# hugofloresgarcia/vampnet

Measured on NVIDIA H100. Metric: codec tokens/sec (coarse 12 steps + c2f 24 steps generate, T=768, 44.1 kHz), higher is better.
Workload: dtype bf16

## Files before the change

vampnet_b200/csrc/api.cu:

```cuda
#include <cuda_bf16.h>
#include <cudaTypedefs.h>

#include <cmath>
#include <cstdarg>
#include <cstdio>
#include <cstring>
#include <map>
#include <memory>
#include <string>
#include <tuple>
#include <vector>

#include "kernels.h"

namespace vnb {

static thread_local std::string g_err;
static thread_local std::string g_tmap_err;

static int fail(const char* fmt, ...) {
  char buf[1024];
  va_list ap;
  va_start(ap, fmt);
  vsnprintf(buf, sizeof(buf), fmt, ap);
  va_end(ap);
  g_err = buf;
  return 1;
}
#define CK(expr)                                                                                   \
  do {                                                                                             \
    cudaError_t _e = (expr);                                                                       \
    if (_e != cudaSuccess) return fail("%s failed: %s (%s:%d)", #expr, cudaGetErrorString(_e), __FILE__, __LINE__); \
  } while (0)

static PFN_cuTensorMapEncodeTiled_v12000 get_encode() {
  static PFN_cuTensorMapEncodeTiled_v12000 fn = nullptr;
  if (fn) return fn;
  void* p = nullptr;
  cudaDriverEntryPointQueryResult q;
  cudaError_t e = cudaGetDriverEntryPoint("cuTensorMapEncodeTiled", &p, cudaEnableDefault, &q);
  if (e != cudaSuccess || q != cudaDriverEntryPointSuccess || !p) {
    g_tmap_err = std::string("cudaGetDriverEntryPoint(cuTensorMapEncodeTiled) failed: ") + cudaGetErrorString(e);
    return nullptr;
  }
  fn = reinterpret_cast<PFN_cuTensorMapEncodeTiled_v12000>(p);
  return fn;
}
const char* tmap_error() { return g_tmap_err.c_str(); }

bool make_tmap_2d(CUtensorMap* tm, const void* base, uint64_t rows, uint64_t cols, uint32_t box_rows,
                  uint32_t box_cols) {
  auto enc = get_encode();
  if (!enc) return false;
  cuuint64_t dims[2] = {cols, rows};
  cuuint64_t strides[1] = {cols * 2};
  cuuint32_t box[2] = {box_cols, box_rows};
  cuuint32_t estr[2] = {1, 1};
  CUresult r = enc(tm, CU_TENSOR_MAP_DATA_TYPE_BFLOAT16, 2, const_cast<void*>(base), dims, strides, box, estr,
                   CU_TENSOR_MAP_INTERLEAVE_NONE, CU_TENSOR_MAP_SWIZZLE_128B, CU_TENSOR_MAP_L2_PROMOTION_L2_256B,
                   CU_TENSOR_MAP_FLOAT_OOB_FILL_NONE);
  if (r != CUDA_SUCCESS) {
    char b[256];
    snprintf(b, sizeof(b), "cuTensorMapEncodeTiled(2d rows=%llu cols=%llu box=%ux%u) -> %d", (unsigned long long)rows,
             (unsigned long long)cols, box_rows, box_cols, (int)r);
    g_tmap_err = b;
    return false;
  }
  return true;
}
bool make_tmap_3d(CUtensorMap* tm, const void* base, uint64_t batch, uint64_t rows, uint64_t cols,
                  uint64_t pitch_elems, uint32_t box_rows, uint32_t box_cols) {
  auto enc = get_encode();
  if (!enc) return false;
  cuuint64_t dims[3] = {cols, rows, batch};
  cuuint64_t strides[2] = {pitch_elems * 2, rows * pitch_elems * 2};
  cuuint32_t box[3] = {box_cols, box_rows, 1};
  cuuint32_t estr[3] = {1, 1, 1};
  CUresult r = enc(tm, CU_TENSOR_MAP_DATA_TYPE_BFLOAT16, 3, const_cast<void*>(base), dims, strides, box, estr,
                   CU_TENSOR_MAP_INTERLEAVE_NONE, CU_TENSOR_MAP_SWIZZLE_128B, CU_TENSOR_MAP_L2_PROMOTION_L2_256B,
                   CU_TENSOR_MAP_FLOAT_OOB_FILL_NONE);
  if (r != CUDA_SUCCESS) {
    char b[256];
    snprintf(b, sizeof(b), "cuTensorMapEncodeTiled(3d batch=%llu rows=%llu cols=%llu pitch=%llu box=%ux%u) -> %d",
             (unsigned long long)batch, (unsigned long long)rows, (unsigned long long)cols,
             (unsigned long long)pitch_elems, box_rows, box_cols, (int)r);
    g_tmap_err = b;
    return false;
  }
  return true;
}

static bool make_gemm_plan(GemmPlan* p, int epi, const void* A, const void* W, int M, int N, int K, void* out,
                           void* out2, const float* bias, int T, int Tpad, const float* ss_in, int ss_parts,
                           float inv_d, float eps, void* out_bf16, float* ss_out) {
  if (N % 256 != 0 || K % 64 != 0 || M < 1) {
    g_tmap_err = "gemm: need N % 256 == 0 and K % 64 == 0";
    return false;
  }
  GemmArgs& a = p->args;
  a.M = M; a.N = N; a.K = K; a.epi = epi; a.out = out; a.out2 = out2; a.bias = bias;
  a.T = T; a.Tpad = Tpad; a.d2 = epi == VNB_EPI_QKV ? (N / 3) * 2 : 0;
  if (ss_in != nullptr) { a.ss_in = ss_in; a.ss_parts = ss_parts; a.inv_d = inv_d; a.eps = eps; }
  a.out_bf16 = reinterpret_cast<__nv_bfloat16*>(out_bf16); a.ss_out = ss_out;
  return make_tmap_2d(&p->tmA, A, M, K, 128, 64) && make_tmap_2d(&p->tmB, W, N, K, 256, 64) &&
         make_tmap_2d(&p->tmBh, W, N, K, 128, 64);
}

bool make_attn_plan(AttnPlan* p, const void* qk, const void* vT, void* out, const float* rel, int sat, int B, int T,
                    int Tpad, int H) {
  const int d = H * 64;
  p->out = out; p->rel = rel; p->sat = sat; p->B = B; p->T = T; p->Tpad = Tpad; p->H = H;
  return make_tmap_3d(&p->tmQ, qk, B, T, 2 * d, 2 * d, 128, 64) && make_tmap_3d(&p->tmK, qk, B, T, 2 * d, 2 * d, 64, 64) &&
         make_tmap_3d(&p->tmVT, vT, B, d, Tpad, Tpad, 64, 64);
}

struct DevBuf {
  void* p = nullptr;
  size_t n = 0;
  ~DevBuf() { if (p) cudaFree(p); }
  cudaError_t alloc(size_t bytes, bool zero = false) {
    n = bytes;
    cudaError_t e = cudaMalloc(&p, bytes ? bytes : 1);
    if (e == cudaSuccess && zero) e = cudaMemset(p, 0, bytes);
    return e;
  }
  template <class T> T* as() const { return reinterpret_cast<T*>(p); }
};

struct Variant {
  int steps = 0;
  bool has_mask = false;
  bool top_p = false;
  int gemm_pair = 0;
  bool fused = false;
  bool adapted = false;
  bool ragged = false;
  bool mixed_steps = false;
  bool split = false;
  bool operator<(const Variant& o) const {
    return std::tie(steps, has_mask, top_p, gemm_pair, fused, adapted, ragged, mixed_steps, split) <
           std::tie(o.steps, o.has_mask, o.top_p, o.gemm_pair, o.fused, o.adapted, o.ragged, o.mixed_steps, o.split);
  }
};

struct Workspace {
  int B = 0, T = 0, Tpad = 0, M = 0;
  unsigned long long last_use = 0;
  DevBuf x, y, qk, vT, att, h, logits, zcur, zorig, tokens, conf, n0, dyn, rowgrp, z_in, mask_in, z_out, ssA, ssB, embA,
      partials;
  DevBuf grp_adapter, lora_u;
  DevBuf frames;
  DevBuf live;
  int embKp = 0;
  int ss_parts = 0;
  std::vector<GemmPlan> qkv, wo, up, down;
  GemmPlan cls, emb;
  GemmPlan cls_sample;
  bool can_fuse = false;
  AttnPlan attn;
  std::map<Variant, cudaGraphExec_t> graphs;
  std::map<Variant, unsigned long long> graph_kernels;
  ~Workspace() { for (auto& kv : graphs) cudaGraphExecDestroy(kv.second); }
};

}

namespace vnb {
enum { FAM_EMBED = 0, FAM_RMSNORM, FAM_GEMM_QKV, FAM_ATTN, FAM_GEMM_O, FAM_GEMM_UP, FAM_GEMM_DOWN, FAM_GEMM_CLS,
       FAM_SAMPLE, FAM_STATE, FAM_LORA_DOWN, FAM_COUNT };
static unsigned long long g_captures = 0;
static unsigned long long g_launches = 0;
void count_launch(unsigned long long n) { g_launches += n; }
struct Profiler {
  bool on = false;
  std::vector<cudaEvent_t> pool;
  std::vector<int> fam;
  size_t used = 0;
  ~Profiler() { for (auto e : pool) cudaEventDestroy(e); }
  void mark(int family, cudaStream_t st) {
    if (!on) return;
    if (used == pool.size()) {
      cudaEvent_t e;
      if (cudaEventCreate(&e) != cudaSuccess) { on = false; return; }
      pool.push_back(e);
      fam.push_back(-1);
    }
// ... 1133 lines not shown
```

vampnet_b200/csrc/common.cuh:

```cuda
#pragma once
#include <cuda.h>
#include <cuda_bf16.h>
#include <cuda_runtime.h>
#include <stdint.h>
#include <stdio.h>

namespace vnb {

__device__ __forceinline__ uint32_t smem_u32(const void* p) {
  return static_cast<uint32_t>(__cvta_generic_to_shared(p));
}
__device__ __forceinline__ uint32_t lane_id() { return threadIdx.x & 31; }

__device__ __forceinline__ bool elect_one() {
  uint32_t pred = 0;
  asm volatile(
      "{\n\t.reg .pred P;\n\t.reg .b32 R;\n\t"
      "elect.sync R|P, 0xffffffff;\n\t"
      "selp.u32 %0, 1, 0, P;\n\t}"
      : "=r"(pred));
  return pred != 0;
}

__device__ __forceinline__ void mbar_init(uint64_t* bar, uint32_t count) {
// ... 91 lines not shown

__device__ __forceinline__ void tma_store_2d(const CUtensorMap* m, const void* src, int c0, int c1) {
  asm volatile("cp.async.bulk.tensor.2d.global.shared::cta.bulk_group [%0, {%2, %3}], [%1];"
               ::"l"(reinterpret_cast<uint64_t>(m)), "r"(smem_u32(src)), "r"(c0), "r"(c1)
               : "memory");
}
__device__ __forceinline__ void bulk_commit() { asm volatile("cp.async.bulk.commit_group;" ::: "memory"); }
template <int N>
__device__ __forceinline__ void bulk_wait_read() {
  asm volatile("cp.async.bulk.wait_group.read %0;" ::"n"(N) : "memory");
}

__device__ __forceinline__ uint32_t cluster_ctarank() {
  uint32_t r;
  asm volatile("mov.u32 %0, %%cluster_ctarank;" : "=r"(r));
  return r;
}
__device__ __forceinline__ void cluster_sync_all() {
  asm volatile("barrier.cluster.arrive.release.aligned;\n\tbarrier.cluster.wait.acquire.aligned;" ::: "memory");
}
__device__ __forceinline__ uint32_t mapa_u32(uint32_t cta_addr, uint32_t rank) {
  uint32_t r;
  asm volatile("mapa.shared::cluster.u32 %0, %1, %2;" : "=r"(r) : "r"(cta_addr), "r"(rank));
  return r;
}
__device__ __forceinline__ void mbar_arrive_cluster(uint32_t cluster_addr) {
  asm volatile("mbarrier.arrive.release.cluster.shared::cluster.b64 _, [%0];" ::"r"(cluster_addr) : "memory");
}
__device__ __forceinline__ bool mbar_try_wait_cluster(uint64_t* bar, uint32_t parity) {
  uint32_t ok;
  asm volatile(
      "{\n\t.reg .pred P;\n\t"
      "mbarrier.try_wait.parity.acquire.cluster.shared::cta.b64 P, [%1], %2, %3;\n\t"
      "selp.u32 %0, 1, 0, P;\n\t}"
      : "=r"(ok)
      : "r"(smem_u32(bar)), "r"(parity), "r"(100000u)
      : "memory");
  return ok != 0;
}
__device__ __forceinline__ void mbar_wait_cluster(uint64_t* bar, uint32_t parity) {
  if (mbar_try_wait_cluster(bar, parity)) return;
  const uint64_t t0 = global_timer_ns();
  while (!mbar_try_wait_cluster(bar, parity))
    if (global_timer_ns() - t0 > VNB_WAIT_TIMEOUT_NS) __trap();
}
__device__ __forceinline__ void tma_load_2d_mc(void* dst, const CUtensorMap* m, uint64_t* bar, int c0, int c1,
                                               uint16_t cta_mask) {
  asm volatile(
      "cp.async.bulk.tensor.2d.shared::cluster.global.mbarrier::complete_tx::bytes.multicast::cluster"
      " [%0], [%1, {%3, %4}], [%2], %5;"
      ::"r"(smem_u32(dst)), "l"(reinterpret_cast<uint64_t>(m)), "r"(smem_u32(bar)), "r"(c0), "r"(c1), "h"(cta_mask)
      : "memory");
}

__device__ __forceinline__ uint32_t pack_bf16x2(float lo, float hi) {
  __nv_bfloat162 v = __floats2bfloat162_rn(lo, hi);
  return *reinterpret_cast<uint32_t*>(&v);
}
__device__ __forceinline__ float fast_exp2(float x) {
  float y;
  asm volatile("ex2.approx.ftz.f32 %0, %1;" : "=f"(y) : "f"(x));
  return y;
}
__device__ __forceinline__ float lds_f32(uint32_t addr) {
  float v;
  asm volatile("ld.shared.f32 %0, [%1];" : "=f"(v) : "r"(addr));
  return v;
}
__device__ __forceinline__ void sts_f32(uint32_t addr, float v) {
  asm volatile("st.shared.f32 [%0], %1;" ::"r"(addr), "f"(v) : "memory");
}
__device__ __forceinline__ void sts_u32(uint32_t addr, uint32_t v) {
  asm volatile("st.shared.b32 [%0], %1;" ::"r"(addr), "r"(v) : "memory");
}
__device__ __forceinline__ float4 lds_f4(uint32_t addr) {
  float4 v;
  asm volatile("ld.shared.v4.f32 {%0, %1, %2, %3}, [%4];" : "=f"(v.x), "=f"(v.y), "=f"(v.z), "=f"(v.w) : "r"(addr));
  return v;
}
__device__ __forceinline__ uint2 lds_u2(uint32_t addr) {
  uint2 v;
  asm volatile("ld.shared.v2.b32 {%0, %1}, [%2];" : "=r"(v.x), "=r"(v.y) : "r"(addr));
  return v;
}
__device__ __forceinline__ void sts_f4(uint32_t addr, float4 v) {
  asm volatile("st.shared.v4.f32 [%0], {%1, %2, %3, %4};" ::"r"(addr), "f"(v.x), "f"(v.y), "f"(v.z), "f"(v.w)
               : "memory");
}
__device__ __forceinline__ void sts_v4(uint32_t addr, uint32_t a, uint32_t b, uint32_t c, uint32_t d) {
  asm volatile("st.shared.v4.b32 [%0], {%1, %2, %3, %4};" ::"r"(addr), "r"(a), "r"(b), "r"(c), "r"(d) : "memory");
}
__device__ __forceinline__ float warp_max(float v) {
#pragma unroll
  for (int o = 16; o > 0; o >>= 1) v = fmaxf(v, __shfl_xor_sync(0xffffffffu, v, o));
  return v;
}
__device__ __forceinline__ float warp_sum(float v) {
#pragma unroll
  for (int o = 16; o > 0; o >>= 1) v += __shfl_xor_sync(0xffffffffu, v, o);
  return v;
}

__device__ __forceinline__ void philox4x32_10(uint32_t c0, uint32_t c1, uint32_t c2, uint32_t c3, uint32_t k0,
                                              uint32_t k1, uint32_t (&out)[4]) {
#pragma unroll
  for (int r = 0; r < 10; ++r) {
    const uint32_t hi0 = __umulhi(0xD2511F53u, c0), lo0 = 0xD2511F53u * c0;
    const uint32_t hi1 = __umulhi(0xCD9E8D57u, c2), lo1 = 0xCD9E8D57u * c2;
    const uint32_t n0 = hi1 ^ c1 ^ k0, n2 = hi0 ^ c3 ^ k1;
    c0 = n0; c1 = lo1; c2 = n2; c3 = lo0;
    k0 += 0x9E3779B9u;
    k1 += 0xBB67AE85u;
  }
  out[0] = c0; out[1] = c1; out[2] = c2; out[3] = c3;
}
__device__ __forceinline__ float u01(uint32_t x) { return (static_cast<float>(x >> 9) + 0.5f) * 1.1920928955078125e-07f; }

}
```

vampnet_b200/csrc/gemm_wgmma.cu:

```cuda
#include <stdlib.h>

#include "common.cuh"
#include "kernels.h"
#include "wgmma.cuh"

#ifndef VNB_GEMM_PAIR_DEFAULT
#define VNB_GEMM_PAIR_DEFAULT false
#endif

namespace vnb {

constexpr int BM = 128, BN = 256, BK = 64, STAGES = 4;
constexpr int A_BYTES = BM * BK * 2;
constexpr int B_BYTES = BN * BK * 2;
constexpr int STAGE_BYTES = A_BYTES + B_BYTES;
constexpr int SBIAS_BYTES = BN * 4;
constexpr int RING_BYTES = STAGES * STAGE_BYTES;
constexpr int ACC_PITCH = BN + 1;
static_assert(BM * ACC_PITCH * 4 <= RING_BYTES, "the accumulator tile overlays the ring");
static_assert(BM * ACC_PITCH * 4 + 4 * BM + 16 + 32 * BM <= RING_BYTES, "the adapted epilogue's row table follows it");
constexpr int GEMM_SMEM = RING_BYTES + SBIAS_BYTES + 1024  + 256 ;
static_assert(GEMM_SMEM <= 227 * 1024, "H100: at most 227 KiB of shared memory per block");
constexpr int GEMM_THREADS = 256 + 32;
template <int EPI> constexpr int gemm_epi_warps() { return (EPI == VNB_EPI_RESID || EPI == VNB_EPI_SAMPLE) ? 8 : 4; }
// ... 381 lines not shown
              for (int j4 = 0; j4 < 8; ++j4) {
                const float4 b4 = lds_f4(sb4 + 16u * (c * 8 + j4));
                const float bj[4] = {b4.x, b4.y, b4.z, b4.w};
#pragma unroll
                for (int j = 0; j < 4; ++j) {
                  const float x = __fadd_rn(__fmul_rn(__uint_as_float(v[j4 * 4 + j]), rs), bj[j]);
                  run += fast_exp2(__fmaf_rn(x, c1, c0));
                  if (run > target && found < 0) { found = c * 32 + j4 * 4 + j; xc = x; }
                }
              }
            }
            if (found >= 0) cand = found;
            else xc = mx;
          }
          if (active)
            g.partials[(static_cast<size_t>(row) * Cp + cp) * (g.V >> 7) + (v0 >> 7)] =
                make_float4(mx, ssum, xc, __uint_as_float(static_cast<uint32_t>(v0 + cand) |
                                                          (static_cast<uint32_t>(v0 + am) << 16)));
        }
      } else if constexpr (EPI == VNB_EPI_RESID || EPI == VNB_EPI_BIAS_F32) {
        const bool fused_out = g.out_bf16 != nullptr;
        constexpr int CSTEP = kWide ? 2 : 1;
        float ssacc[8];
#pragma unroll
        for (int i = 0; i < 8; ++i) ssacc[i] = 0.f;
        auto process = [&](int c, const float4 (&add)[8]) {
          if (fused_out) drain_f32<true>(g, qaddr, rs, lane, row_base, n0, c, add, ssacc);
          else drain_f32<false>(g, qaddr, rs, lane, row_base, n0, c, add, ssacc);
        };
        float4 addA[8], addB[8];
        prefetch_addend<EPI>(g, lane, row_base, n0 + half * 32, addA);
#pragma unroll 1
        for (int c = half; c < BN / 32; c += 2 * CSTEP) {
          prefetch_addend<EPI>(g, lane, row_base, n0 + (c + CSTEP) * 32, addB);
          process(c, addA);
          if (c + 2 * CSTEP < BN / 32) prefetch_addend<EPI>(g, lane, row_base, n0 + (c + 2 * CSTEP) * 32, addA);
          process(c + CSTEP, addB);
        }
        if (fused_out) {
#pragma unroll
          for (int it = 0; it < 8; ++it) {
            float v = ssacc[it];
            v += __shfl_xor_sync(0xffffffffu, v, 1);
            v += __shfl_xor_sync(0xffffffffu, v, 2);
            v += __shfl_xor_sync(0xffffffffu, v, 4);
            const int rr = row_base + it * 4 + (lane >> 3);
            const int part = (n0 / BN) * (kWide ? 2 : 1) + half;
            if ((lane & 7) == 0 && rr < g.M) g.ss_out[static_cast<size_t>(part) * g.M + rr] = v;
          }
        }
      } else {
#pragma unroll 1
        for (int c = 0; c < BN / 32; ++c) {
          const int col0 = n0 + c * 32;
          if constexpr (EPI == VNB_EPI_QKV) {
            if (col0 >= g.d2) {
              uint32_t v[32];
              acc_ld_x32(t_addr + 4u * (c * 32), v);
              if (row_ok) {
                const int d = g.N - g.d2;
                __nv_bfloat16* o = reinterpret_cast<__nv_bfloat16*>(g.out2) +
                                   (static_cast<size_t>(b_idx) * d + (col0 - g.d2)) * g.Tpad + t_idx;
                const bool pad = g.frames != nullptr && t_idx >= __ldg(g.frames + b_idx);
#pragma unroll
                for (int j = 0; j < 32; ++j)
                  o[static_cast<size_t>(j) * g.Tpad] =
                      pad ? __float2bfloat16_rn(0.f) : __float2bfloat16_rn(__uint_as_float(v[j]) * rs);
              }
              continue;
            }
          }
          drain_bf16<false>(reinterpret_cast<__nv_bfloat16*>(g.out), EPI == VNB_EPI_BF16 ? g.N : g.d2, g.M, qaddr, rs, lane,
                            row_base, c * 32, col0);
        }
      }
    }
  }
  if constexpr (PAIR) cluster_sync_all();
}

constexpr int PERS_EPI_WARPS = 3;
constexpr int PERS_THREADS = 256 + 32 * PERS_EPI_WARPS + 32;
template <int EPI> constexpr int pers_stages() { return EPI == VNB_EPI_QKV ? 3 : STAGES; }
template <int EPI> constexpr int pers_out_bytes() { return EPI == VNB_EPI_QKV ? BM * BN * 2 : BM * (BN / 2) * 2; }
template <int EPI>
constexpr int pers_smem() {
  return pers_stages<EPI>() * STAGE_BYTES + pers_out_bytes<EPI>() + 4 * BM  + 1024  +
         128 ;
}
static_assert(pers_smem<VNB_EPI_GEGLU>() <= 227 * 1024, "H100: at most 227 KiB of shared memory per block");
static_assert(pers_smem<VNB_EPI_QKV>() <= 227 * 1024, "H100: at most 227 KiB of shared memory per block");
static_assert((2 * STAGES + 2) * 8 <= 128, "the barriers fit their slot");

template <int PITCH>
__device__ __forceinline__ uint32_t stage_off(int r, int w) {
  return static_cast<uint32_t>(r * PITCH + (((w >> 2) ^ (r & 7)) << 4) + ((w & 3) << 2));
}

template <int EPI>
__global__ void __launch_bounds__(PERS_THREADS, 1)
gemm_persistent_kernel(const __grid_constant__ CUtensorMap tmA, const __grid_constant__ CUtensorMap tmB,
                       const GemmArgs g) {
  constexpr int NS = pers_stages<EPI>();
  constexpr int RING = NS * STAGE_BYTES;
  constexpr int OUT_BYTES = pers_out_bytes<EPI>();
  extern __shared__ uint8_t smem_raw[];
  uint8_t* smem = reinterpret_cast<uint8_t*>((reinterpret_cast<uintptr_t>(smem_raw) + 1023) & ~uintptr_t(1023));
  const uint32_t stage_tile = smem_u32(smem + RING);
  float* srs = reinterpret_cast<float*>(smem + RING + OUT_BYTES);
  uint64_t* full_bar = reinterpret_cast<uint64_t*>(smem + RING + OUT_BYTES + 4 * BM);
  uint64_t* empty_bar = full_bar + NS;
  uint64_t* out_full = empty_bar + NS;
  uint64_t* out_free = out_full + 1;

  const int warp = threadIdx.x >> 5;
  const int lane = threadIdx.x & 31;
  const int num_n = g.N / BN;
  const int num_kb = g.K / BK;
  const int tiles = ((live_rows(g) + BM - 1) / BM) * num_n;
  constexpr int kProducer = 8 + PERS_EPI_WARPS;

  if (warp == kProducer && lane == 0) {
    tma_prefetch_desc(&tmA);
    tma_prefetch_desc(&tmB);
    for (int s = 0; s < NS; ++s) {
      mbar_init(&full_bar[s], 1);
      mbar_init(&empty_bar[s], 8);
    }
    mbar_init(out_full, 256);
    mbar_init(out_free, 32 * PERS_EPI_WARPS);
    mbar_fence_init();
  }
  __syncthreads();

  if (warp == kProducer) {
    if (lane == 0) {
      int stage = 0;
      uint32_t phase = 0;
      for (int tile = blockIdx.x; tile < tiles; tile += gridDim.x) {
        const int m0 = (tile / num_n) * BM, n0 = (tile % num_n) * BN;
        for (int kb = 0; kb < num_kb; ++kb) {
          mbar_wait(&empty_bar[stage], phase ^ 1);
          uint8_t* sa = smem + stage * STAGE_BYTES;
          mbar_expect_tx(&full_bar[stage], STAGE_BYTES);
          tma_load_2d(sa, &tmA, &full_bar[stage], kb * BK, m0);
          tma_load_2d(sa + A_BYTES, &tmB, &full_bar[stage], kb * BK, n0);
          if (++stage == NS) { stage = 0; phase ^= 1; }
        }
      }
    }
    __syncwarp();
  } else if (warp < 8) {
    int stage = 0;
    uint32_t phase = 0;
    uint32_t it = 0;
    const int r = (warp >> 2) * 64 + (warp & 3) * 16 + (lane >> 2);
    for (int tile = blockIdx.x; tile < tiles; tile += gridDim.x, ++it) {
      float acc[128];
      gemm_mainloop<NS>(acc, smem, full_bar, num_kb, warp >> 2, stage, phase, [&](int s) {
        if (lane == 0) mbar_arrive(&empty_bar[s]);
      });
      mbar_wait(out_free, it & 1u);
      const float rs0 = srs[r], rs1 = srs[r + 8];
      if constexpr (EPI == VNB_EPI_GEGLU) {
#pragma unroll
        for (int i = 0; i < 16; ++i) {
          float x[4];
#pragma unroll
          for (int k = 0; k < 4; ++k) {
            const float rsr = k < 2 ? rs0 : rs1;
            x[k] = acc[4 * i + k] * rsr;
            x[k] = x[k] * gelu_tanh(acc[4 * (i + 16) + k] * rsr);
          }
          const int w = 4 * i + (lane & 3);
          sts_u32(stage_tile + stage_off<256>(r, w), pack_bf16x2(x[0], x[1]));
          sts_u32(stage_tile + stage_off<256>(r + 8, w), pack_bf16x2(x[2], x[3]));
        }
      } else if ((tile % num_n) * BN < g.d2) {
#pragma unroll
        for (int i = 0; i < 32; ++i) {
          const int w = 4 * i + (lane & 3);
          sts_u32(stage_tile + stage_off<512>(r, w), pack_bf16x2(acc[4 * i] * rs0, acc[4 * i + 1] * rs0));
          sts_u32(stage_tile + stage_off<512>(r + 8, w), pack_bf16x2(acc[4 * i + 2] * rs1, acc[4 * i + 3] * rs1));
        }
      } else {
        const bool odd = (lane >> 2) & 1;
#pragma unroll
        for (int i = 0; i < 32; ++i) {
          const int c = 8 * i + 2 * (lane & 3) + (odd ? 1 : 0);
#pragma unroll
          for (int h = 0; h < 2; ++h) {
            const float rsr = h ? rs1 : rs0;
            const uint32_t own = pack_bf16x2(acc[4 * i + 2 * h] * rsr, acc[4 * i + 2 * h + 1] * rsr);
            const uint32_t peer = __shfl_xor_sync(0xffffffffu, own, 4);
            sts_u32(stage_tile + stage_off<256>(c, (r + 8 * h) >> 1),
                    odd ? __byte_perm(peer, own, 0x7632) : __byte_perm(own, peer, 0x5410));
          }
        }
      }
      mbar_arrive(out_full);
    }
  } else {
    const int e = warp - 8;
    __nv_bfloat16* const out = reinterpret_cast<__nv_bfloat16*>(g.out);
    const int pitch = EPI == VNB_EPI_GEGLU ? g.N / 2 : g.d2;
    auto row_scales = [&](int tile) {
      if (tile < tiles) {
        const int m0 = (tile / num_n) * BM;
        for (int j = e * 32 + lane; j < BM; j += 32 * PERS_EPI_WARPS) srs[j] = row_scale(g, m0 + j);
      }
      mbar_arrive(out_free);
    };
    row_scales(blockIdx.x);
    uint32_t it = 0;
    for (int tile = blockIdx.x; tile < tiles; tile += gridDim.x, ++it) {
      const int m0 = (tile / num_n) * BM, n0 = (tile % num_n) * BN;
      mbar_wait(out_full, it & 1u);
      if constexpr (EPI == VNB_EPI_GEGLU) {
#pragma unroll 4
        for (int u = e; u < BM / 2; u += PERS_EPI_WARPS) {
          const int rr = 2 * u + (lane >> 4);
          const float4 v = lds_f4(stage_tile + stage_off<256>(rr, 4 * (lane & 15)));
          if (m0 + rr < g.M)
            *reinterpret_cast<float4*>(out + static_cast<size_t>(m0 + rr) * pitch + (n0 >> 1) + 8 * (lane & 15)) = v;
        }
      } else if (n0 < g.d2) {
#pragma unroll 4
        for (int rr = e; rr < BM; rr += PERS_EPI_WARPS) {
          const float4 v = lds_f4(stage_tile + stage_off<512>(rr, 4 * lane));
          if (m0 + rr < g.M)
            *reinterpret_cast<float4*>(out + static_cast<size_t>(m0 + rr) * pitch + n0 + 8 * lane) = v;
        }
      } else {
        const int d = g.N - g.d2;
        uint16_t* const vt = reinterpret_cast<uint16_t*>(g.out2) + static_cast<size_t>(n0 - g.d2) * g.Tpad;
        size_t off[4];
        bool ok[4];
        int bk[4];
        uint32_t keep[2] = {0xffffffffu, 0xffffffffu};
#pragma unroll
        for (int k = 0; k < 4; ++k) {
          const int m = m0 + 4 * lane + k;
          bk[k] = m / g.T;
          const int t = m - bk[k] * g.T;
          ok[k] = m < g.M;
          off[k] = static_cast<size_t>(bk[k]) * d * g.Tpad + t;
          if (ok[k] && g.frames != nullptr && t >= __ldg(g.frames + bk[k])) keep[k >> 1] &= (k & 1) ? 0xffffu : 0xffff0000u;
        }
        const bool wide = ok[3] && bk[3] == bk[0] && (off[0] & 3) == 0 && (g.Tpad & 3) == 0 &&
                          (reinterpret_cast<uintptr_t>(g.out2) & 7) == 0;
#pragma unroll 2
        for (int c = e; c < BN; c += PERS_EPI_WARPS) {
          uint2 v = lds_u2(stage_tile + stage_off<256>(c, 2 * lane));
          v.x &= keep[0];
          v.y &= keep[1];
          uint16_t* const o = vt + static_cast<size_t>(c) * g.Tpad;
          if (wide) {
            *reinterpret_cast<uint2*>(o + off[0]) = v;
          } else {
#pragma unroll
            for (int k = 0; k < 4; ++k) {
              const uint32_t w = k < 2 ? v.x : v.y;
              if (ok[k]) o[off[k]] = static_cast<uint16_t>((k & 1) ? (w >> 16) : w);
            }
          }
        }
      }
      row_scales(tile + gridDim.x);
    }
  }
}

static int g_gemm_pair = -1;
void set_gemm_pair(int on) { g_gemm_pair = on ? 1 : 0; }
static bool gemm_pair_enabled() {
  if (g_gemm_pair < 0) {
    const char* e = getenv("VNB_GEMM_PAIR");
    g_gemm_pair = e != nullptr ? (e[0] == '1') : (VNB_GEMM_PAIR_DEFAULT ? 1 : 0);
  }
  return g_gemm_pair == 1;
}
int get_gemm_pair() { return gemm_pair_enabled() ? 1 : 0; }

static int g_max_clusters[6][64];
template <int EPI>
static cudaError_t init_epi() {
  static PerDeviceOnce once;
  int dev;
  if (!once.need(&dev)) return cudaSuccess;
  cudaError_t e = cudaFuncSetAttribute(gemm_wgmma_kernel<EPI, false>, cudaFuncAttributeMaxDynamicSharedMemorySize, GEMM_SMEM);
  if (e != cudaSuccess) return e;
  e = cudaFuncSetAttribute(gemm_wgmma_kernel<EPI, true>, cudaFuncAttributeMaxDynamicSharedMemorySize, GEMM_SMEM);
  if (e != cudaSuccess) return e;
  if constexpr (EPI == VNB_EPI_QKV || EPI == VNB_EPI_RESID || EPI == VNB_EPI_GEGLU) {
    e = cudaFuncSetAttribute(gemm_wgmma_kernel<EPI, false, true>, cudaFuncAttributeMaxDynamicSharedMemorySize, GEMM_SMEM);
    if (e != cudaSuccess) return e;
    e = cudaFuncSetAttribute(gemm_wgmma_kernel<EPI, true, true>, cudaFuncAttributeMaxDynamicSharedMemorySize, GEMM_SMEM);
    if (e != cudaSuccess) return e;
  }
  if constexpr (EPI == VNB_EPI_GEGLU || EPI == VNB_EPI_QKV) {
    e = cudaFuncSetAttribute(gemm_persistent_kernel<EPI>, cudaFuncAttributeMaxDynamicSharedMemorySize, pers_smem<EPI>());
    if (e != cudaSuccess) return e;
  }
  if constexpr (EPI == VNB_EPI_SAMPLE) {
    e = cudaFuncSetAttribute(gemm_wgmma_kernel<EPI, false, false, true>, cudaFuncAttributeMaxDynamicSharedMemorySize,
                             GEMM_SMEM);
    if (e != cudaSuccess) return e;
    e = cudaFuncSetAttribute(gemm_wgmma_kernel<EPI, true, false, true>, cudaFuncAttributeMaxDynamicSharedMemorySize,
                             GEMM_SMEM);
    if (e != cudaSuccess) return e;
  }
  cudaLaunchConfig_t q = {};
  q.gridDim = dim3(2 * device_sm_count());
  q.blockDim = dim3(GEMM_THREADS);
  q.dynamicSmemBytes = GEMM_SMEM;
  cudaLaunchAttribute qa[1];
  qa[0].id = cudaLaunchAttributeClusterDimension;
  qa[0].val.clusterDim.x = 2; qa[0].val.clusterDim.y = 1; qa[0].val.clusterDim.z = 1;
  q.attrs = qa; q.numAttrs = 1;
  int n = 0;
  e = cudaOccupancyMaxActiveClusters(&n, gemm_wgmma_kernel<EPI, true>, &q);
  if (e != cudaSuccess || n <= 0) { (void)cudaGetLastError(); n = device_sm_count() / 2; }
  if (dev >= 0 && dev < 64) g_max_clusters[EPI][dev] = n;
  once.mark(dev);
  return cudaSuccess;
}
cudaError_t prepare_gemm() {
  cudaError_t e;
  if ((e = init_epi<VNB_EPI_BF16>()) != cudaSuccess) return e;
  if ((e = init_epi<VNB_EPI_QKV>()) != cudaSuccess) return e;
  if ((e = init_epi<VNB_EPI_RESID>()) != cudaSuccess) return e;
  if ((e = init_epi<VNB_EPI_GEGLU>()) != cudaSuccess) return e;
  if ((e = init_epi<VNB_EPI_BIAS_F32>()) != cudaSuccess) return e;
  return init_epi<VNB_EPI_SAMPLE>();
}

int get_gemm_max_clusters() {
  int dev = 0;
  cudaGetDevice(&dev);
  if (prepare_gemm() != cudaSuccess || dev < 0 || dev >= 64) return 0;
  return g_max_clusters[VNB_EPI_RESID][dev];
}

template <int EPI, bool ADAPT = false, bool SPLIT = false>
static cudaError_t launch_epi(const GemmPlan& p, const GemmArgs& g, cudaStream_t st) {
  cudaError_t e = init_epi<EPI>();
  if (e != cudaSuccess) return e;
  if (gemm_pair_enabled()) {
    const int clusters = ((g.M + 2 * BM - 1) / (2 * BM)) * (g.N / BN);
    cudaLaunchConfig_t cfg = {};
    cfg.gridDim = dim3(2 * clusters);
    cfg.blockDim = dim3(GEMM_THREADS);
    cfg.dynamicSmemBytes = GEMM_SMEM;
    cfg.stream = st;
    cudaLaunchAttribute attr[1];
    attr[0].id = cudaLaunchAttributeClusterDimension;
    attr[0].val.clusterDim.x = 2; attr[0].val.clusterDim.y = 1; attr[0].val.clusterDim.z = 1;
    cfg.attrs = attr; cfg.numAttrs = 1;
    return cudaLaunchKernelEx(&cfg, gemm_wgmma_kernel<EPI, true, ADAPT, SPLIT>, p.tmA, p.tmBh, g);
  }
  const int tiles = ((g.M + BM - 1) / BM) * (g.N / BN);
  if constexpr ((EPI == VNB_EPI_GEGLU || EPI == VNB_EPI_QKV) && !ADAPT) {
    const int grid = tiles < device_sm_count() ? tiles : device_sm_count();
    gemm_persistent_kernel<EPI><<<grid, PERS_THREADS, pers_smem<EPI>(), st>>>(p.tmA, p.tmB, g);
    return cudaGetLastError();
  }
  gemm_wgmma_kernel<EPI, false, ADAPT, SPLIT><<<tiles, GEMM_THREADS, GEMM_SMEM, st>>>(p.tmA, p.tmB, g);
  return cudaGetLastError();
}

cudaError_t launch_gemm(const GemmPlan& p, cudaStream_t st) {
  GemmArgs g = p.args;
  if (g.epi != VNB_EPI_QKV) g.frames = nullptr;
  if (g.lora.table != nullptr) {
    if (!g.lora.grp_adapter || !g.lora.rowgrp || !g.lora.u || g.lora.rows_per_grp < 1) return cudaErrorInvalidValue;
    switch (g.epi) {
      case VNB_EPI_QKV: return launch_epi<VNB_EPI_QKV, true>(p, g, st);
      case VNB_EPI_RESID: return launch_epi<VNB_EPI_RESID, true>(p, g, st);
      case VNB_EPI_GEGLU: return launch_epi<VNB_EPI_GEGLU, true>(p, g, st);
      default: return cudaErrorInvalidValue;
    }
  }
  switch (g.epi) {
    case VNB_EPI_BF16: return launch_epi<VNB_EPI_BF16>(p, g, st);
    case VNB_EPI_QKV: return launch_epi<VNB_EPI_QKV>(p, g, st);
    case VNB_EPI_RESID: return launch_epi<VNB_EPI_RESID>(p, g, st);
    case VNB_EPI_GEGLU: return launch_epi<VNB_EPI_GEGLU>(p, g, st);
    case VNB_EPI_BIAS_F32: return launch_epi<VNB_EPI_BIAS_F32>(p, g, st);
    case VNB_EPI_SAMPLE:
      if (!g.zcur || !g.dyn || !g.rowgrp || !g.partials || !g.bias || g.V % 128 != 0 || g.V > 1024) return cudaErrorInvalidValue;
      if (p.sample_split) {
        if (!g.out) return cudaErrorInvalidValue;
        return launch_epi<VNB_EPI_SAMPLE, false, true>(p, g, st);
      }
      return launch_epi<VNB_EPI_SAMPLE>(p, g, st);
    default: return cudaErrorInvalidValue;
  }
}

__global__ void gemm_ref_kernel(const __nv_bfloat16* A, const __nv_bfloat16* W, int M, int N, int K, float* out) {
  const int n = blockIdx.x * blockDim.x + threadIdx.x;
  const int m = blockIdx.y;
  if (n >= N || m >= M) return;
  float acc = 0.f;
  for (int k = 0; k < K; ++k)
    acc += __bfloat162float(A[static_cast<size_t>(m) * K + k]) * __bfloat162float(W[static_cast<size_t>(n) * K + k]);
  out[static_cast<size_t>(m) * N + n] = acc;
}
cudaError_t launch_gemm_ref(const void* A, const void* W, int M, int N, int K, float* out, cudaStream_t st) {
  dim3 grid((N + 127) / 128, M);
  gemm_ref_kernel<<<grid, 128, 0, st>>>(reinterpret_cast<const __nv_bfloat16*>(A),
                                        reinterpret_cast<const __nv_bfloat16*>(W), M, N, K, out);
  return cudaGetLastError();
}

}
```

vampnet_b200/csrc/kernels.h:

```cpp
#pragma once
#include <cuda.h>
#include <cuda_bf16.h>
#include <cuda_runtime.h>
#include <stdint.h>

#include "../../include/vampnet_b200.h"

namespace vnb {

struct PerDeviceOnce {
  unsigned long long done = 0;
  bool need(int* dev_out) {
    int dev = 0;
    cudaGetDevice(&dev);
    *dev_out = dev;
    return dev >= 64 || !((done >> dev) & 1ull);
  }
  void mark(int dev) { if (dev < 64) done |= 1ull << dev; }
};
inline int device_sm_count() {
  static int sms[64] = {0};
  int dev = 0;
  cudaGetDevice(&dev);
  if (dev >= 64) { int n = 0; cudaDeviceGetAttribute(&n, cudaDevAttrMultiProcessorCount, dev); return n; }
  if (!sms[dev]) cudaDeviceGetAttribute(&sms[dev], cudaDevAttrMultiProcessorCount, dev);
  return sms[dev];
}

void count_launch(unsigned long long n = 1);

bool make_tmap_2d(CUtensorMap* tm, const void* base, uint64_t rows, uint64_t cols, uint32_t box_rows,
                  uint32_t box_cols);
bool make_tmap_3d(CUtensorMap* tm, const void* base, uint64_t batch, uint64_t rows, uint64_t cols,
                  uint64_t pitch_elems, uint32_t box_rows, uint32_t box_cols);
const char* tmap_error();
}
extern "C" int32_t vnb_set_error_cuda(const char* what, int32_t cuda_error);
namespace vnb {

struct SampleDyn;
struct RowGroup {
  int32_t group, first;
};

enum { LORA_QKV = 0, LORA_WO, LORA_W1, LORA_W2, LORA_SLOTS };
struct AdapterDev {
  const float* a[LORA_SLOTS];
  const float* b[LORA_SLOTS];
};
struct AdapterRefs {
  const AdapterDev* table = nullptr;
  const int32_t* grp_adapter = nullptr;
  const RowGroup* rowgrp = nullptr;
  int rows_per_grp = 1;
  int slot = 0, layer = 0;
  float* u = nullptr;
};
cudaError_t launch_lora_down(const void* y, int M, int K, const AdapterRefs& r, const int32_t* live, int T,
                             cudaStream_t st);

struct GemmArgs {
  int M, N, K;
  int epi;
  void* out;
  void* out2;
  const float* bias;
  int T, Tpad;
  int d2;
  __nv_bfloat16* out_bf16;
  float* ss_out;
  const float* ss_in;
  int ss_parts;
  float inv_d, eps;
  const int32_t* zcur;
  const SampleDyn* dyn;
  const RowGroup* rowgrp;
  float4* partials;
  int C, ncc, V, mask_token;
  AdapterRefs lora;
  const int32_t* frames;
  const int32_t* live;
};
struct GemmPlan {
  CUtensorMap tmA, tmB;
  CUtensorMap tmBh;
  bool sample_split = false;
  GemmArgs args{};
};
cudaError_t launch_gemm(const GemmPlan& p, cudaStream_t st);
cudaError_t prepare_gemm();
void set_gemm_pair(int on);
int get_gemm_pair();
int get_gemm_max_clusters();
cudaError_t launch_gemm_ref(const void* A, const void* W, int M, int N, int K, float* out, cudaStream_t st);

struct AttnPlan {
  CUtensorMap tmQ;
  CUtensorMap tmK;
  CUtensorMap tmVT;
  void* out = nullptr;
  const float* rel = nullptr;
  const int32_t* frames = nullptr;
  const int32_t* live = nullptr;
  int sat = 0, B = 0, T = 0, Tpad = 0, H = 0;
};
bool make_attn_plan(AttnPlan* p, const void* qk, const void* vT, void* out, const float* rel, int sat, int B, int T,
                    int Tpad, int H);
cudaError_t launch_attention(const AttnPlan& p, cudaStream_t st);

cudaError_t launch_embed_gather(const int32_t* codes_btc, const float* latents, const float* table, void* A, int M, int T,
                                int C, int V1, int K, int Kp, float* ss, int zero_from, int ss_parts,
                                const int32_t* live, cudaStream_t st);

cudaError_t launch_gen_init(const int64_t* z, const int32_t* mask, int32_t* zcur, int32_t* zorig, int32_t* n0,
                            const RowGroup* rowgrp, int n_groups, int B, int C, int T, int ncc, int mask_token,
                            cudaStream_t st);
cudaError_t launch_gen_finish(const int32_t* tokens, const int32_t* zorig, int64_t* out, int B, int C, int T, int ncc,
                              cudaStream_t st);

struct SampleDyn {
  float inv_temp, gamma, temp_eff;
  int do_sample, is_last, step;
  uint32_t seed_lo, seed_hi;
  float top_p;
};
struct SampleArgs {
  const float* logits;
  int32_t* zcur;
  const int32_t* zorig;
  int32_t* tokens;
  float* conf;
  const int32_t* n0;
  const RowGroup* rowgrp;
  int B, T, C, ncc, V, mask_token;
  const int32_t* live = nullptr;
};
cudaError_t launch_sample_step_dev(const SampleArgs& a, const SampleDyn* dyn_dev, cudaStream_t st, bool use_top_p);
cudaError_t launch_sample_combine_dev(const SampleArgs& a, const void* partials, const SampleDyn* dyn_dev, cudaStream_t st);
cudaError_t launch_remask_dev(const SampleArgs& a, const SampleDyn* dyn_dev, cudaStream_t st);
cudaError_t launch_sample_split_dev(const SampleArgs& a, const void* partials, const SampleDyn* dyn_dev, cudaStream_t st);

struct OnsetGeometry {
  int pre_max = 0, post_max = 0, pre_avg = 0, post_avg = 0, wait = 0, pad = 0;
};
OnsetGeometry onset_geometry(int sr, int hop);
struct OnsetTables {
  const float2* twiddle;
  const float* window;
  const float* mel_w;
  const int32_t* mel_off;
  const int32_t* mel_lo;
  int pre_max, post_max, pre_avg, post_avg, wait, pad;
  float delta;
};
cudaError_t onset_tables(int sr, int hop, OnsetTables* out);
cudaError_t launch_onset_detect(const float* samples, int B, int N, int hop, const OnsetTables& t, float* db_ws,
                                float* env, int32_t* onsets, int32_t* counts, int backtrack, cudaStream_t st);
cudaError_t launch_onset_mask(const int32_t* onsets, const int32_t* counts, int onset_rows, int F, int width,
                              int64_t* mask, int B, int C, int T, cudaStream_t st);
cudaError_t launch_onset_spec(const float* samples, int B, int N, int hop, const OnsetTables& t, float* db,
                              cudaStream_t st);

constexpr int BEAT_MAX_LAGS = 4096;
int beat_lags(int sr, int hop);
struct BeatTables {
  const double* window;
  const double* bpm;
  const double* log2_bpm;
// ... 40 lines not shown
```

Measured before the change: 290,400.

## Route residual-add GEMMs through persistent kernel with TMA-prefetched residual tiles

Residual-epilogue GEMMs (out projection, FFN down) now use the persistent warp-specialized kernel. The producer TMA-loads the fp32 residual tile into the operand ring stages after the K loop. The math warps then add the scaled accumulator in shared memory and write coalesced fp32, bf16 and sum-of-squares outputs. This is meant to overlap the residual read with the mainloop of the next tile and to remove strided global loads, at the cost of extra ring stages per tile and a more intricate barrier protocol.

```diff
diff --git a/vampnet_b200/csrc/api.cu b/vampnet_b200/csrc/api.cu
--- a/vampnet_b200/csrc/api.cu
+++ b/vampnet_b200/csrc/api.cu
@@ -48,25 +48,33 @@
 }
 const char* tmap_error() { return g_tmap_err.c_str(); }
 
-bool make_tmap_2d(CUtensorMap* tm, const void* base, uint64_t rows, uint64_t cols, uint32_t box_rows,
-                  uint32_t box_cols) {
+static bool encode_2d(CUtensorMap* tm, CUtensorMapDataType type, uint64_t elem_bytes, const void* base, uint64_t rows,
+                      uint64_t cols, uint32_t box_rows, uint32_t box_cols) {
   auto enc = get_encode();
   if (!enc) return false;
   cuuint64_t dims[2] = {cols, rows};
-  cuuint64_t strides[1] = {cols * 2};
+  cuuint64_t strides[1] = {cols * elem_bytes};
   cuuint32_t box[2] = {box_cols, box_rows};
   cuuint32_t estr[2] = {1, 1};
-  CUresult r = enc(tm, CU_TENSOR_MAP_DATA_TYPE_BFLOAT16, 2, const_cast<void*>(base), dims, strides, box, estr,
-                   CU_TENSOR_MAP_INTERLEAVE_NONE, CU_TENSOR_MAP_SWIZZLE_128B, CU_TENSOR_MAP_L2_PROMOTION_L2_256B,
-                   CU_TENSOR_MAP_FLOAT_OOB_FILL_NONE);
+  CUresult r = enc(tm, type, 2, const_cast<void*>(base), dims, strides, box, estr, CU_TENSOR_MAP_INTERLEAVE_NONE,
+                   CU_TENSOR_MAP_SWIZZLE_128B, CU_TENSOR_MAP_L2_PROMOTION_L2_256B, CU_TENSOR_MAP_FLOAT_OOB_FILL_NONE);
   if (r != CUDA_SUCCESS) {
     char b[256];
-    snprintf(b, sizeof(b), "cuTensorMapEncodeTiled(2d rows=%llu cols=%llu box=%ux%u) -> %d", (unsigned long long)rows,
-             (unsigned long long)cols, box_rows, box_cols, (int)r);
+    snprintf(b, sizeof(b), "cuTensorMapEncodeTiled(2d %s rows=%llu cols=%llu box=%ux%u) -> %d",
+             elem_bytes == 4 ? "fp32" : "bf16", (unsigned long long)rows, (unsigned long long)cols, box_rows, box_cols,
+             (int)r);
     g_tmap_err = b;
     return false;
   }
   return true;
+}
+bool make_tmap_2d(CUtensorMap* tm, const void* base, uint64_t rows, uint64_t cols, uint32_t box_rows,
+                  uint32_t box_cols) {
+  return encode_2d(tm, CU_TENSOR_MAP_DATA_TYPE_BFLOAT16, 2, base, rows, cols, box_rows, box_cols);
+}
+bool make_tmap_2d_f32(CUtensorMap* tm, const void* base, uint64_t rows, uint64_t cols, uint32_t box_rows,
+                      uint32_t box_cols) {
+  return encode_2d(tm, CU_TENSOR_MAP_DATA_TYPE_FLOAT32, 4, base, rows, cols, box_rows, box_cols);
 }
 bool make_tmap_3d(CUtensorMap* tm, const void* base, uint64_t batch, uint64_t rows, uint64_t cols,
                   uint64_t pitch_elems, uint32_t box_rows, uint32_t box_cols) {
@@ -102,6 +110,7 @@
   a.T = T; a.Tpad = Tpad; a.d2 = epi == VNB_EPI_QKV ? (N / 3) * 2 : 0;
   if (ss_in != nullptr) { a.ss_in = ss_in; a.ss_parts = ss_parts; a.inv_d = inv_d; a.eps = eps; }
   a.out_bf16 = reinterpret_cast<__nv_bfloat16*>(out_bf16); a.ss_out = ss_out;
+  if (epi == VNB_EPI_RESID && !make_tmap_2d_f32(&p->tmR, out, M, N, 128, 32)) return false;
   return make_tmap_2d(&p->tmA, A, M, K, 128, 64) && make_tmap_2d(&p->tmB, W, N, K, 256, 64) &&
          make_tmap_2d(&p->tmBh, W, N, K, 128, 64);
 }
diff --git a/vampnet_b200/csrc/common.cuh b/vampnet_b200/csrc/common.cuh
--- a/vampnet_b200/csrc/common.cuh
+++ b/vampnet_b200/csrc/common.cuh
@@ -197,6 +197,9 @@
   uint2 v;
   asm volatile("ld.shared.v2.b32 {%0, %1}, [%2];" : "=r"(v.x), "=r"(v.y) : "r"(addr));
   return v;
+}
+__device__ __forceinline__ void sts_u2(uint32_t addr, uint32_t a, uint32_t b) {
+  asm volatile("st.shared.v2.b32 [%0], {%1, %2};" ::"r"(addr), "r"(a), "r"(b) : "memory");
 }
 __device__ __forceinline__ void sts_f4(uint32_t addr, float4 v) {
   asm volatile("st.shared.v4.f32 [%0], {%1, %2, %3, %4};" ::"r"(addr), "f"(v.x), "f"(v.y), "f"(v.z), "f"(v.w)
diff --git a/vampnet_b200/csrc/gemm_wgmma.cu b/vampnet_b200/csrc/gemm_wgmma.cu
--- a/vampnet_b200/csrc/gemm_wgmma.cu
+++ b/vampnet_b200/csrc/gemm_wgmma.cu
@@ -487,7 +487,9 @@
 constexpr int PERS_EPI_WARPS = 3;
 constexpr int PERS_THREADS = 256 + 32 * PERS_EPI_WARPS + 32;
 template <int EPI> constexpr int pers_stages() { return EPI == VNB_EPI_QKV ? 3 : STAGES; }
-template <int EPI> constexpr int pers_out_bytes() { return EPI == VNB_EPI_QKV ? BM * BN * 2 : BM * (BN / 2) * 2; }
+template <int EPI> constexpr int pers_out_bytes() {
+  return EPI == VNB_EPI_QKV ? BM * BN * 2 : EPI == VNB_EPI_RESID ? 0 : BM * (BN / 2) * 2;
+}
 template <int EPI>
 constexpr int pers_smem() {
   return pers_stages<EPI>() * STAGE_BYTES + pers_out_bytes<EPI>() + 4 * BM  + 1024  +
@@ -496,6 +498,12 @@
 static_assert(pers_smem<VNB_EPI_GEGLU>() <= 227 * 1024, "H100: at most 227 KiB of shared memory per block");
 static_assert(pers_smem<VNB_EPI_QKV>() <= 227 * 1024, "H100: at most 227 KiB of shared memory per block");
 static_assert((2 * STAGES + 2) * 8 <= 128, "the barriers fit their slot");
+constexpr int RES_BOX_COLS = 32;
+constexpr int RES_BOX_BYTES = BM * RES_BOX_COLS * 4;
+constexpr int RES_BOXES = BN / RES_BOX_COLS;
+constexpr int RES_PER_STAGE = STAGE_BYTES / RES_BOX_BYTES;
+constexpr int RES_STAGES = (RES_BOXES + RES_PER_STAGE - 1) / RES_PER_STAGE;
+static_assert(RES_PER_STAGE == 3 && RES_STAGES == 3 && RES_STAGES < STAGES, "the residual rows take 3 of the 4 stages");
 
 template <int PITCH>
 __device__ __forceinline__ uint32_t stage_off(int r, int w) {
@@ -505,7 +513,7 @@
 template <int EPI>
 __global__ void __launch_bounds__(PERS_THREADS, 1)
 gemm_persistent_kernel(const __grid_constant__ CUtensorMap tmA, const __grid_constant__ CUtensorMap tmB,
-                       const GemmArgs g) {
+                       const __grid_constant__ CUtensorMap tmR, const GemmArgs g) {
   constexpr int NS = pers_stages<EPI>();
   constexpr int RING = NS * STAGE_BYTES;
   constexpr int OUT_BYTES = pers_out_bytes<EPI>();
@@ -528,6 +536,7 @@
   if (warp == kProducer && lane == 0) {
     tma_prefetch_desc(&tmA);
     tma_prefetch_desc(&tmB);
+    if constexpr (EPI == VNB_EPI_RESID) tma_prefetch_desc(&tmR);
     for (int s = 0; s < NS; ++s) {
       mbar_init(&full_bar[s], 1);
       mbar_init(&empty_bar[s], 8);
@@ -551,6 +560,17 @@
           tma_load_2d(sa, &tmA, &full_bar[stage], kb * BK, m0);
           tma_load_2d(sa + A_BYTES, &tmB, &full_bar[stage], kb * BK, n0);
           if (++stage == NS) { stage = 0; phase ^= 1; }
+        }
+        if constexpr (EPI == VNB_EPI_RESID) {
+          for (int b0 = 0; b0 < RES_BOXES; b0 += RES_PER_STAGE) {
+            const int nb = RES_BOXES - b0 < RES_PER_STAGE ? RES_BOXES - b0 : RES_PER_STAGE;
+            mbar_wait(&empty_bar[stage], phase ^ 1);
+            mbar_expect_tx(&full_bar[stage], nb * RES_BOX_BYTES);
+            for (int b = 0; b < nb; ++b)
+              tma_load_2d(smem + stage * STAGE_BYTES + b * RES_BOX_BYTES, &tmR, &full_bar[stage],
+                          n0 + (b0 + b) * RES_BOX_COLS, m0);
+            if (++stage == NS) { stage = 0; phase ^= 1; }
+          }
         }
       }
     }
@@ -581,6 +601,70 @@
           sts_u32(stage_tile + stage_off<256>(r, w), pack_bf16x2(x[0], x[1]));
           sts_u32(stage_tile + stage_off<256>(r + 8, w), pack_bf16x2(x[2], x[3]));
         }
+      } else if constexpr (EPI == VNB_EPI_RESID) {
+        const int m0 = (tile / num_n) * BM, n0 = (tile % num_n) * BN;
+        const bool fused_out = g.out_bf16 != nullptr;
+        const uint32_t foff = static_cast<uint32_t>(r * 128 + ((((lane & 3) >> 1) ^ (lane >> 2)) << 4) + (lane & 1) * 8);
+        const int crow = (warp >> 2) * 64 + (warp & 3) * 16 + (lane >> 3);
+        const uint32_t coff = static_cast<uint32_t>(crow * 128 + (((lane & 7) ^ (crow & 7)) << 4));
+        const size_t o0 = static_cast<size_t>(m0 + crow) * g.N + n0 + 4 * (lane & 7);
+        float* const xo = reinterpret_cast<float*>(g.out) + o0;
+        float ssacc[2][4];
+#pragma unroll
+        for (int h = 0; h < 2; ++h)
+#pragma unroll
+          for (int it = 0; it < 4; ++it) ssacc[h][it] = 0.f;
+        uint32_t sres = 0;
+#pragma unroll
+        for (int b = 0; b < RES_BOXES; ++b) {
+          if (b % RES_PER_STAGE == 0) {
+            mbar_wait(&full_bar[stage], phase);
+            sres = smem_u32(smem + stage * STAGE_BYTES);
+          }
+          const uint32_t box = sres + (b % RES_PER_STAGE) * RES_BOX_BYTES;
+#pragma unroll
+          for (int j = 0; j < 4; ++j) {
+            const int i = 4 * b + j;
+            const uint32_t a = box + (foff ^ (32u * j));
+            const uint2 x0 = lds_u2(a), x1 = lds_u2(a + 8 * 128);
+            sts_u2(a, __float_as_uint(__fadd_rn(__fmul_rn(acc[4 * i], rs0), __uint_as_float(x0.x))),
+                   __float_as_uint(__fadd_rn(__fmul_rn(acc[4 * i + 1], rs0), __uint_as_float(x0.y))));
+            sts_u2(a + 8 * 128, __float_as_uint(__fadd_rn(__fmul_rn(acc[4 * i + 2], rs1), __uint_as_float(x1.x))),
+                   __float_as_uint(__fadd_rn(__fmul_rn(acc[4 * i + 3], rs1), __uint_as_float(x1.y))));
+          }
+          __syncwarp();
+#pragma unroll
+          for (int it = 0; it < 4; ++it) {
+            const float4 o = lds_f4(box + (coff ^ (64u * (it & 1))) + it * 512);
+            if (m0 + crow + 4 * it < g.M) {
+              *reinterpret_cast<float4*>(xo + static_cast<size_t>(4 * it) * g.N + b * RES_BOX_COLS) = o;
+              if (fused_out) {
+                *reinterpret_cast<uint2*>(g.out_bf16 + o0 + static_cast<size_t>(4 * it) * g.N + b * RES_BOX_COLS) =
+                    make_uint2(pack_bf16x2(o.x, o.y), pack_bf16x2(o.z, o.w));
+                ssacc[b & 1][it] = __fadd_rn(ssacc[b & 1][it], sumsq4(o.x, o.y, o.z, o.w));
+              }
+            }
+          }
+          if (b % RES_PER_STAGE == RES_PER_STAGE - 1 || b == RES_BOXES - 1) {
+            fence_proxy_async_smem();
+            __syncwarp();
+            if (lane == 0) mbar_arrive(&empty_bar[stage]);
+            if (++stage == NS) { stage = 0; phase ^= 1; }
+          }
+        }
+        if (fused_out) {
+#pragma unroll
+          for (int h = 0; h < 2; ++h)
+#pragma unroll
+            for (int it = 0; it < 4; ++it) {
+              float v = ssacc[h][it];
+              v += __shfl_xor_sync(0xffffffffu, v, 1);
+              v += __shfl_xor_sync(0xffffffffu, v, 2);
+              v += __shfl_xor_sync(0xffffffffu, v, 4);
+              const int rr = m0 + crow + 4 * it;
+              if ((lane & 7) == 0 && rr < g.M) g.ss_out[static_cast<size_t>((n0 / BN) * 2 + h) * g.M + rr] = v;
+            }
+        }
       } else if ((tile % num_n) * BN < g.d2) {
 #pragma unroll
         for (int i = 0; i < 32; ++i) {
@@ -629,6 +713,7 @@
           if (m0 + rr < g.M)
             *reinterpret_cast<float4*>(out + static_cast<size_t>(m0 + rr) * pitch + (n0 >> 1) + 8 * (lane & 15)) = v;
         }
+      } else if constexpr (EPI == VNB_EPI_RESID) {
       } else if (n0 < g.d2) {
 #pragma unroll 4
         for (int rr = e; rr < BM; rr += PERS_EPI_WARPS) {
@@ -703,7 +788,7 @@
     e = cudaFuncSetAttribute(gemm_wgmma_kernel<EPI, true, true>, cudaFuncAttributeMaxDynamicSharedMemorySize, GEMM_SMEM);
     if (e != cudaSuccess) return e;
   }
-  if constexpr (EPI == VNB_EPI_GEGLU || EPI == VNB_EPI_QKV) {
+  if constexpr (EPI == VNB_EPI_GEGLU || EPI == VNB_EPI_QKV || EPI == VNB_EPI_RESID) {
     e = cudaFuncSetAttribute(gemm_persistent_kernel<EPI>, cudaFuncAttributeMaxDynamicSharedMemorySize, pers_smem<EPI>());
     if (e != cudaSuccess) return e;
   }
@@ -765,9 +850,9 @@
     return cudaLaunchKernelEx(&cfg, gemm_wgmma_kernel<EPI, true, ADAPT, SPLIT>, p.tmA, p.tmBh, g);
   }
   const int tiles = ((g.M + BM - 1) / BM) * (g.N / BN);
-  if constexpr ((EPI == VNB_EPI_GEGLU || EPI == VNB_EPI_QKV) && !ADAPT) {
+  if constexpr ((EPI == VNB_EPI_GEGLU || EPI == VNB_EPI_QKV || EPI == VNB_EPI_RESID) && !ADAPT) {
     const int grid = tiles < device_sm_count() ? tiles : device_sm_count();
-    gemm_persistent_kernel<EPI><<<grid, PERS_THREADS, pers_smem<EPI>(), st>>>(p.tmA, p.tmB, g);
+    gemm_persistent_kernel<EPI><<<grid, PERS_THREADS, pers_smem<EPI>(), st>>>(p.tmA, p.tmB, p.tmR, g);
     return cudaGetLastError();
   }
   gemm_wgmma_kernel<EPI, false, ADAPT, SPLIT><<<tiles, GEMM_THREADS, GEMM_SMEM, st>>>(p.tmA, p.tmB, g);
diff --git a/vampnet_b200/csrc/kernels.h b/vampnet_b200/csrc/kernels.h
--- a/vampnet_b200/csrc/kernels.h
+++ b/vampnet_b200/csrc/kernels.h
@@ -31,6 +31,8 @@
 
 bool make_tmap_2d(CUtensorMap* tm, const void* base, uint64_t rows, uint64_t cols, uint32_t box_rows,
                   uint32_t box_cols);
+bool make_tmap_2d_f32(CUtensorMap* tm, const void* base, uint64_t rows, uint64_t cols, uint32_t box_rows,
+                      uint32_t box_cols);
 bool make_tmap_3d(CUtensorMap* tm, const void* base, uint64_t batch, uint64_t rows, uint64_t cols,
                   uint64_t pitch_elems, uint32_t box_rows, uint32_t box_cols);
 const char* tmap_error();
@@ -84,6 +86,7 @@
 struct GemmPlan {
   CUtensorMap tmA, tmB;
   CUtensorMap tmBh;
+  CUtensorMap tmR{};
   bool sample_split = false;
   GemmArgs args{};
 };
```

Result: faster. 294,200, median of 6 (+1.3%).
